# microsoft/vision-longformer

Measured on NVIDIA H100. Metric: images/sec ViL-Small 224x224 training, higher is better.
Workload: dtype bf16

## Files before the change

vision_longformer_b200/csrc/vil_common.cuh:

```cuda
#pragma once
#include <cuda_runtime.h>
#include <cuda_bf16.h>
#include <cuda_fp16.h>
#include <stdint.h>
#include "../../include/vil_attn.h"

namespace vil {

struct Geo {
  int B, H, D;
  int nx, ny, w, g, exact, mode;
  int padx, pady, mx, my;
  int Nloc, N, w2;
  int npc;
  int noffs;
  int offR[9], offC[9];
  int has_bias;
  float scale;
  float drop_p, drop_scale;
  uint32_t drop_thresh;
  uint32_t seed_lo, seed_hi, drop_off;
};

inline long long ws_off_delta_g(const Geo& g) { return ((long long)g.B * g.H * g.Nloc + 63) & ~63LL; }
// ... 62 lines not shown
      return;
    }
  }
#pragma unroll
  for (int c = 0; c < CNT; ++c)
    if (c0 + c < D) row[c0 + c] = ElemTraits<T>::from_f(r[c]);
}

__device__ __forceinline__ uint4 philox(const Geo& g, uint32_t c0, uint32_t c1, uint32_t c2) {
  uint32_t x0 = c0, x1 = c1, x2 = c2, x3 = g.drop_off, k0 = g.seed_lo, k1 = g.seed_hi;
#pragma unroll
  for (int r = 0; r < 10; ++r) {
    const uint32_t lo0 = 0xD2511F53u * x0, hi0 = __umulhi(0xD2511F53u, x0);
    const uint32_t lo1 = 0xCD9E8D57u * x2, hi1 = __umulhi(0xCD9E8D57u, x2);
    x0 = hi1 ^ x1 ^ k0; x1 = lo1; x2 = hi0 ^ x3 ^ k1; x3 = lo0;
    k0 += 0x9E3779B9u; k1 += 0xBB67AE85u;
  }
  return make_uint4(x0, x1, x2, x3);
}
__device__ __forceinline__ uint32_t philox_word(const uint4& x, uint32_t w) {
  return w == 0 ? x.x : w == 1 ? x.y : w == 2 ? x.z : x.w;
}
__device__ __forceinline__ bool drop_keep(const Geo& g, uint32_t row, uint32_t col, uint32_t sid) {
  return philox_word(philox(g, col >> 2, row, sid), col & 3) >= g.drop_thresh;
}
__device__ __forceinline__ void drop_keep2(const Geo& g, uint32_t row, uint32_t col, uint32_t sid, bool& k0, bool& k1) {
  const uint4 x = philox(g, col >> 2, row, sid);
  const uint32_t w = col & 3;
  k0 = philox_word(x, w) >= g.drop_thresh;
  const uint32_t u1 = w == 3 ? philox(g, (col >> 2) + 1, row, sid).x : philox_word(x, w + 1);
  k1 = u1 >= g.drop_thresh;
}

__device__ __forceinline__ float warp_sum(float v) {
#pragma unroll
  for (int o = 16; o > 0; o >>= 1) v += __shfl_xor_sync(0xffffffffu, v, o);
  return v;
}

}
```

vision_longformer_b200/csrc/vil_sm90.cuh:

```cuda
#pragma once
#include <cuda_bf16.h>
#include <cuda_fp16.h>
#include <stdint.h>

namespace sm90 {

__device__ __forceinline__ uint32_t smem_u32(const void* p) { return (uint32_t)__cvta_generic_to_shared(p); }

__host__ __device__ constexpr int core_off(int r, int c, int K) { return (((r >> 3) * (K >> 3) + (c >> 3)) << 6) + ((r & 7) << 3) + (c & 7); }

__device__ __forceinline__ uint64_t make_desc(uint32_t addr, uint32_t lbo, uint32_t sbo) {
  return (uint64_t)((addr >> 4) & 0x3FFF) | (uint64_t)(lbo >> 4) << 16 | (uint64_t)(sbo >> 4) << 32;
}
__device__ __forceinline__ uint64_t desc(const void* tile, int K, int k16) {
  return make_desc(smem_u32(tile) + k16 * 256, 128, (K >> 3) * 128);
}
__device__ __forceinline__ uint64_t desc_mn(const void* tile, int N, int k16) {
  return make_desc(smem_u32(tile) + k16 * N * 32, N * 16, 128);
}

__device__ __forceinline__ void cp_async16(void* dst, const void* src, int n) {
  asm volatile("cp.async.cg.shared.global [%0], [%1], 16, %2;" ::"r"(smem_u32(dst)), "l"(src), "r"(n) : "memory");
}
__device__ __forceinline__ void cp_async4(void* dst, const void* src) {
  asm volatile("cp.async.ca.shared.global [%0], [%1], 4;" ::"r"(smem_u32(dst)), "l"(src) : "memory");
}
__device__ __forceinline__ void cp_async_commit() { asm volatile("cp.async.commit_group;" ::: "memory"); }
template <int N>
__device__ __forceinline__ void cp_async_wait() { asm volatile("cp.async.wait_group %0;" ::"n"(N) : "memory"); }

__device__ __forceinline__ void wg_fence() { asm volatile("wgmma.fence.sync.aligned;" ::: "memory"); }
__device__ __forceinline__ void wg_commit() { asm volatile("wgmma.commit_group.sync.aligned;" ::: "memory"); }
__device__ __forceinline__ void wg_wait0() { asm volatile("wgmma.wait_group.sync.aligned 0;" ::: "memory"); }
__device__ __forceinline__ void fence_proxy_async() { asm volatile("fence.proxy.async.shared::cta;" ::: "memory"); }
template <int R>
__device__ __forceinline__ void reg_fence(float (&d)[R]) {
#pragma unroll
  for (int i = 0; i < R; ++i) asm volatile("" : "+f"(d[i])::"memory");
}

__device__ __forceinline__ void wgmma_ss_bf16_n16(float (&d)[8], uint64_t a, uint64_t b, uint32_t acc) {
  asm volatile(
      "{\n\t.reg .pred p;\n\tsetp.ne.b32 p, %10, 0;\n\t"
      "wgmma.mma_async.sync.aligned.m64n16k16.f32.bf16.bf16 {%0,%1,%2,%3,%4,%5,%6,%7}, %8, %9, p, 1, 1, 0, 0;\n\t}"
      : "+f"(d[0]), "+f"(d[1]), "+f"(d[2]), "+f"(d[3]), "+f"(d[4]), "+f"(d[5]), "+f"(d[6]), "+f"(d[7])
      : "l"(a), "l"(b), "r"(acc));
}
__device__ __forceinline__ void wgmma_rs_bf16_n16(float (&d)[8], const uint32_t (&a)[4], uint64_t b, uint32_t acc) {
  asm volatile(
      "{\n\t.reg .pred p;\n\tsetp.ne.b32 p, %13, 0;\n\t"
      "wgmma.mma_async.sync.aligned.m64n16k16.f32.bf16.bf16 {%0,%1,%2,%3,%4,%5,%6,%7}, {%8,%9,%10,%11}, %12, p, 1, 1, 1;\n\t}"
      : "+f"(d[0]), "+f"(d[1]), "+f"(d[2]), "+f"(d[3]), "+f"(d[4]), "+f"(d[5]), "+f"(d[6]), "+f"(d[7])
      : "r"(a[0]), "r"(a[1]), "r"(a[2]), "r"(a[3]), "l"(b), "r"(acc));
}
__device__ __forceinline__ void wgmma_ss_f16_n16(float (&d)[8], uint64_t a, uint64_t b, uint32_t acc) {
// ... 96 lines not shown
```

vision_longformer_b200/csrc/vil_wgmma.cuh:

```cuda
#pragma once
#include "vil_common.cuh"
#include "vil_sm90.cuh"

namespace vil {
namespace wg {

constexpr int kThreads = 128;

struct Cta { int b, h, R, C, piece; };

__device__ __forceinline__ Cta decode(const Geo& g, int bid) {
  Cta c;
  c.piece = bid % g.npc; bid /= g.npc;
  c.C = bid % g.my; bid /= g.my;
  c.R = bid % g.mx; bid /= g.mx;
  c.h = bid % g.H;
  c.b = bid / g.H;
  return c;
}

__device__ __forceinline__ int acc_row(int i) { return ((threadIdx.x >> 5) << 4) + ((threadIdx.x & 31) >> 2) + (((i >> 1) & 1) << 3); }
__device__ __forceinline__ int acc_col(int i) { return ((i >> 2) << 3) + ((threadIdx.x & 3) << 1) + (i & 1); }

constexpr int kStages = 3;

template <typename T, int HD>
__device__ __forceinline__ void stage_row(T* tile, const T* base, long long st, long long tok, int row, int half, int D) {
  constexpr int HH = HD / 2;
  const T* src = base + (tok < 0 ? 0 : tok * st);
#pragma unroll
  for (int g8 = 0; g8 < HH / 8; ++g8) {
    const int c = half * HH + g8 * 8;
    const bool in = tok >= 0 && c < D;
    sm90::cp_async16(tile + sm90::core_off(row, c, HD), in ? src + c : base, in ? 16 : 0);
  }
}

template <typename T>
__device__ __forceinline__ void to_a_frag(const float (&s)[32], int kk, uint32_t (&a)[4]) {
  a[0] = sm90::pack2<T>(s[8 * kk + 0], s[8 * kk + 1]);
  a[1] = sm90::pack2<T>(s[8 * kk + 2], s[8 * kk + 3]);
  a[2] = sm90::pack2<T>(s[8 * kk + 4], s[8 * kk + 5]);
  a[3] = sm90::pack2<T>(s[8 * kk + 6], s[8 * kk + 7]);
}

template <typename TO, int HD>
__device__ __forceinline__ void store_rows(const float (&acc)[HD / 2], int e, TO* row, int D, float mul) {
  const int c0 = (threadIdx.x & 3) << 1;
#pragma unroll
  for (int j = 0; j < HD / 8; ++j) {
    const int col = 8 * j + c0;
    if (col < D) row[col] = ElemTraits<TO>::from_f(acc[4 * j + 2 * e] * mul);
    if (col + 1 < D) row[col + 1] = ElemTraits<TO>::from_f(acc[4 * j + 2 * e + 1] * mul);
  }
}

__device__ __forceinline__ void drop_key_piece(float (&x)[32], const Geo& geo, const uint32_t (&row)[2], int cbase, uint32_t sid,
                                               float mul) {
  uint32_t keep = 0;
#pragma unroll 1
  for (int i = 0; i < 32; i += 2) {
    bool k0, k1;
    drop_keep2(geo, (i & 2) ? row[1] : row[0], (uint32_t)(cbase + acc_col(i)), sid, k0, k1);
    keep |= ((uint32_t)k0 | ((uint32_t)k1 << 1)) << i;
  }
#pragma unroll
  for (int i = 0; i < 32; ++i) x[i] = (keep >> i) & 1u ? x[i] * mul : 0.f;
}

__device__ __forceinline__ void drop_rows(const Geo& geo, int R, int C, int piece, uint32_t (&row)[2]) {
#pragma unroll
  for (int e = 0; e < 2; ++e) {
    const int l = piece * 64 + acc_row(2 * e);
    row[e] = (uint32_t)((R * geo.w + l / geo.w) * geo.ny + C * geo.w + l % geo.w);
  }
}

struct Visit {
  int r, c;
  int dR, dC;
  int cut;
  int oi;
};

__device__ __forceinline__ int visit_list(const Geo& geo, int R, int C, int sgn, Visit* vl) {
  int n = 0;
  for (int oi = 0; oi < geo.noffs; ++oi) {
    const int dR = geo.offR[oi], dC = geo.offC[oi];
    int r = R + sgn * dR, c = C + sgn * dC;
    if (geo.exact == -1) { r = (r + geo.mx) % geo.mx; c = (c + geo.my) % geo.my; }
    else if (r < 0 || r >= geo.mx || c < 0 || c >= geo.my) continue;
    const int qR = sgn > 0 ? R : r, qC = sgn > 0 ? C : c;
    if (threadIdx.x == 0) vl[n] = Visit{r, c, dR, dC, (qR + dR == geo.mx - 1) | ((qC + dC == geo.my - 1) << 1), oi};
    ++n;
  }
  return n;
}

__device__ __forceinline__ int drop_col_base(const Geo& geo, const Visit* vl, int ngp, int pi) {
  if (pi < ngp) return pi * 64;
  const int vi = (pi - ngp) / geo.npc;
  return geo.g + vl[vi].oi * geo.w2 + (pi - ngp - vi * geo.npc) * 64;
}

struct SlotWalk {
  int vi, pj, kr, kc;
  int r0, c0, dr, dc;
  __device__ __forceinline__ SlotWalk(const Geo& geo, int slot)
      : vi(0), pj(0), r0(slot / geo.w), c0(slot % geo.w), dr(64 / geo.w), dc(64 % geo.w) { kr = r0; kc = c0; }
  __device__ __forceinline__ void next(const Geo& geo) {
    if (++pj == geo.npc) { pj = 0; ++vi; kr = r0; kc = c0; return; }
    kr += dr; kc += dc;
    if (kc >= geo.w) { kc -= geo.w; ++kr; }
  }
};

__device__ __forceinline__ void chunk_key(const Geo& geo, const Visit& v, int kr, int kc, long long& tok, bool& ok, int& vr, int& vc) {
  const int w = geo.w;
  const int ar = v.r * w + kr, ac = v.c * w + kc;
  const bool real = (ar < geo.nx) && (ac < geo.ny);
  if (geo.exact == -1)
    ok = !(((v.cut & 1) && (kr >= w - geo.padx)) || ((v.cut & 2) && (kc >= w - geo.pady)));
  else
    ok = real;
  tok = (ok && real) ? geo.g + (long long)ar * geo.ny + ac : -1;
  vr = v.dR * w + kr; vc = v.dC * w + kc;
}

__device__ __forceinline__ void key_slot(const Geo& geo, const Visit* vl, int ngp, int pi, int slot, SlotWalk& wk, int& gk,
                                         long long& tok, bool& ok, int& vr, int& vc) {
  gk = -1; tok = -1; ok = false; vr = 0; vc = 0;
  if (pi < ngp) {
    const int t = pi * 64 + slot;
    if (t < geo.g) { gk = t; tok = t; ok = true; }
    return;
  }
  if (wk.kr < geo.w) chunk_key(geo, vl[wk.vi], wk.kr, wk.kc, tok, ok, vr, vc);
  wk.next(geo);
}

struct KeyCols {
  float* bias;
  int* tix;
  short* kr;
  short* kc;
};
struct QRows {
  int qr[2], qc[2];
  bool ok[2];
};

__device__ __forceinline__ QRows query_rows(const Geo& geo, int R, int C, int piece) {
  QRows q;
  const int w = geo.w;
#pragma unroll
  for (int e = 0; e < 2; ++e) {
    const int l = piece * 64 + acc_row(2 * e);
    const bool in = l < geo.w2;
    q.qr[e] = in ? l / w : 0; q.qc[e] = in ? l % w : 0;
    q.ok[e] = in && (R * w + q.qr[e] < geo.nx) && (C * w + q.qc[e] < geo.ny);
  }
  return q;
}

__device__ __forceinline__ void stage_key_cols(const Geo& geo, const KeyCols& kc, int h, const float* __restrict__ g2l, int gk,
                                               bool ok, int vr, int vc) {
  const int slot = threadIdx.x >> 1;
  float bias = ok ? 0.f : -INFINITY;
  if (gk >= 0 && geo.has_bias) bias = g2l[((long long)geo.H + h) * geo.g + gk];
  kc.bias[slot] = bias;
  kc.tix[slot] = vr * (4 * geo.w - 1) + vc;
  kc.kr[slot] = (short)vr;
  kc.kc[slot] = (short)vc;
}

__device__ __forceinline__ void row_tix(const Geo& geo, const QRows& q, int (&tb)[2]) {
  const int w = geo.w, tw = 4 * w - 1;
  tb[0] = (q.qr[0] + 2 * w - 1) * tw + q.qc[0] + 2 * w - 1;
  tb[1] = (q.qr[1] + 2 * w - 1) * tw + q.qc[1] + 2 * w - 1;
}

template <bool RPE, bool WIN>
__device__ __forceinline__ float key_score(const Geo& geo, const KeyCols& kc, const float* tab, const QRows& q, const int (&tb)[2],
                                           int e, int j, int gl, float s, int& bidx) {
  float bias = kc.bias[j];
  bidx = -1;
  if (RPE && j >= gl) { bidx = tb[e] - kc.tix[j]; bias += tab[bidx]; }
  if (WIN && (abs(q.qr[e] - kc.kr[j]) > geo.w || abs(q.qc[e] - kc.kc[j]) > geo.w)) return -INFINITY;
  return fmaf(geo.scale, s, bias);
}

__device__ __forceinline__ int key_epilogue(const Geo& geo) { return (geo.has_bias ? 2 : 0) | (geo.exact == 1 ? 1 : 0); }

template <bool RPE, bool WIN>
__device__ __forceinline__ void fwd_scores(float (&s)[32], float (&mx)[2], const Geo& geo, const KeyCols& kc, const float* tab,
                                           const QRows& q, int gl) {
  int tb[2] = {0, 0};
  if (RPE) row_tix(geo, q, tb);
#pragma unroll
  for (int i = 0; i < 32; ++i) {
    const int e = (i >> 1) & 1;
    int bidx;
    s[i] = key_score<RPE, WIN>(geo, kc, tab, q, tb, e, acc_col(i), gl, s[i], bidx);
    mx[e] = fmaxf(mx[e], s[i]);
  }
}

template <bool RPE, bool WIN>
__device__ __forceinline__ void dq_scores(float (&s)[32], const float (&dp)[32], const Geo& geo, const KeyCols& kc,
                                          const float* tab, const QRows& q, int gl, const float (&lse_r)[2],
                                          const float (&del_r)[2], float* __restrict__ d_table, int h) {
  int tb[2] = {0, 0};
  if (RPE) row_tix(geo, q, tb);
#pragma unroll
  for (int i = 0; i < 32; ++i) {
    const int e = (i >> 1) & 1;
    int bidx;
    const float val = key_score<RPE, WIN>(geo, kc, tab, q, tb, e, acc_col(i), gl, s[i], bidx);
    const float ds = __expf(val - lse_r[e]) * (dp[i] - del_r[e]);
    if (RPE && d_table != nullptr && bidx >= 0 && q.ok[e] && val != -INFINITY)
      atomicAdd(d_table + (long long)bidx * geo.H + h, ds);
    s[i] = ds;
  }
}

constexpr size_t kKeyCols = 64 * (4 + 4 + 2 + 2);
constexpr size_t kQueryCols = 64 * (4 + 4 + 4 + 2 + 2 + 1);
constexpr size_t kVisits = 9 * sizeof(Visit);
__host__ __device__ constexpr size_t query_cols_bytes(bool drop) { return kQueryCols + (drop ? 64 * sizeof(int) : 0); }

__device__ __forceinline__ KeyCols key_cols(unsigned char* meta, int stage) {
  KeyCols kc;
  kc.bias = reinterpret_cast<float*>(meta + stage * kKeyCols);
  kc.tix = reinterpret_cast<int*>(kc.bias + 64);
  kc.kr = reinterpret_cast<short*>(kc.tix + 64);
  kc.kc = kc.kr + 64;
  return kc;
}

template <int HD> struct FwdSmem {
  static constexpr size_t tiles = (1 + 2 * kStages) * 64 * HD * 2;
  static size_t total(int tabn) { return (tiles + kStages * kKeyCols + kVisits + (size_t)tabn * 4 + 15) & ~size_t(15); }
};
template <int HD> struct DqSmem {
  static constexpr size_t tiles = (2 + 2 * kStages) * 64 * HD * 2;
  static size_t total(int tabn) { return (tiles + kStages * kKeyCols + kVisits + (size_t)tabn * 4 + 15) & ~size_t(15); }
};
template <int HD> struct DkvSmem {
  static constexpr size_t tiles = (2 + 2 * kStages) * 64 * HD * 2;
  static size_t total(int tabn, bool drop = false) {
    return (tiles + kStages * query_cols_bytes(drop) + kVisits + 64 * sizeof(int) + (size_t)tabn * 4 + 15) & ~size_t(15);
  }
};

template <typename T, int HD>
__device__ __forceinline__ void issue_key_piece(const Geo& geo, int pi, int npieces, int ngp, const Visit* vl, SlotWalk& wk,
                                                T* ring, unsigned char* meta, const T* kb, long long kst, const T* vb,
                                                long long vst, int h, const float* __restrict__ g2l) {
  if (pi < npieces) {
    const int slot = threadIdx.x >> 1, half = threadIdx.x & 1, st = pi % kStages;
    int gk, vr, vc;
    long long tok;
    bool ok;
    key_slot(geo, vl, ngp, pi, slot, wk, gk, tok, ok, vr, vc);
    T* Ks = ring + st * 2 * 64 * HD;
    stage_row<T, HD>(Ks, kb, kst, tok, slot, half, geo.D);
    stage_row<T, HD>(Ks + 64 * HD, vb, vst, tok, slot, half, geo.D);
    if (half == 0) stage_key_cols(geo, key_cols(meta, st), h, g2l, gk, ok, vr, vc);
  }
  sm90::cp_async_commit();
}

__device__ __forceinline__ void ring_wait() {
  sm90::cp_async_wait<kStages - 2>();
  sm90::fence_proxy_async();
  __syncthreads();
}

template <typename T, int HD, typename TO, bool DROP = false>
__global__ void __launch_bounds__(kThreads, HD <= 32 ? 5 : 3)
wg_fwd_local(Geo geo, T4 q, T4 k, T4 v, T4 o, float* __restrict__ lse, const float* __restrict__ table,
             const float* __restrict__ g2l) {
  constexpr int HH = HD / 2, TILE = 64 * HD;
  using W64 = sm90::Wg<T, 64>;
  using WHD = sm90::Wg<T, HD>;
  extern __shared__ __align__(128) unsigned char smem_raw[];
  T* Qs = reinterpret_cast<T*>(smem_raw);
  T* ring = Qs + TILE;
  unsigned char* meta = reinterpret_cast<unsigned char*>(ring + 2 * kStages * TILE);
  Visit* vl = reinterpret_cast<Visit*>(meta + kStages * kKeyCols);
  float* tab = reinterpret_cast<float*>(vl + 9);
  const int tabn = geo.has_bias ? (4 * geo.w - 1) * (4 * geo.w - 1) : 0;

  const Cta cid = decode(geo, blockIdx.x);
  const int b = cid.b, h = cid.h, R = cid.R, C = cid.C;
  const int tid = threadIdx.x, slot = tid >> 1, half = tid & 1;
  const int w = geo.w, D = geo.D;
  for (int i = tid; i < tabn; i += kThreads) tab[i] = table[(long long)i * geo.H + h];
  {
    const int l = cid.piece * 64 + slot;
    const int r = R * w + l / w, c = C * w + l % w;
    const bool real = l < geo.w2 && r < geo.nx && c < geo.ny;
    stage_row<T, HD>(Qs, row_ptr<T>(q, b, h, 0), q.st, real ? (long long)r * geo.ny + c : -1, slot, half, D);
  }
  float m[2] = {-INFINITY, -INFINITY}, lsum[2] = {0.f, 0.f};
  float oacc[HH];
#pragma unroll
  for (int i = 0; i < HH; ++i) oacc[i] = 0.f;

  const int ngp = (geo.g + 63) / 64, npieces = ngp + visit_list(geo, R, C, 1, vl) * geo.npc;
  const int epi = key_epilogue(geo);
  const T* kb = row_ptr<T>(k, b, h, 0);
  const T* vb = row_ptr<T>(v, b, h, 0);
  SlotWalk wk(geo, slot);
  __syncthreads();
#pragma unroll
  for (int p = 0; p < kStages - 1; ++p)
    issue_key_piece<T, HD>(geo, p, npieces, ngp, vl, wk, ring, meta, kb, k.st, vb, v.st, h, g2l);
  for (int pi = 0; pi < npieces; ++pi) {
    ring_wait();
    issue_key_piece<T, HD>(geo, pi + kStages - 1, npieces, ngp, vl, wk, ring, meta, kb, k.st, vb, v.st, h, g2l);
    const int st = pi % kStages;
    const T* Ks = ring + st * 2 * TILE;
    const T* Vs = Ks + TILE;
    const KeyCols kcol = key_cols(meta, st);
    float s[32];
    sm90::wg_fence();
#pragma unroll
    for (int kk = 0; kk < HD / 16; ++kk) W64::ss(s, sm90::desc(Qs, HD, kk), sm90::desc(Ks, HD, kk), kk > 0);
    sm90::wg_commit();
    sm90::wg_wait0();
    sm90::reg_fence(s);
    float mx[2] = {-INFINITY, -INFINITY};
    const int gl = geo.g - pi * 64;
    switch (epi) {
      case 0: fwd_scores<false, false>(s, mx, geo, kcol, tab, query_rows(geo, R, C, cid.piece), gl); break;
      case 1: fwd_scores<false, true>(s, mx, geo, kcol, tab, query_rows(geo, R, C, cid.piece), gl); break;
      case 2: fwd_scores<true, false>(s, mx, geo, kcol, tab, query_rows(geo, R, C, cid.piece), gl); break;
      default: fwd_scores<true, true>(s, mx, geo, kcol, tab, query_rows(geo, R, C, cid.piece), gl); break;
    }
    float corr[2];
#pragma unroll
    for (int e = 0; e < 2; ++e) {
      mx[e] = fmaxf(mx[e], __shfl_xor_sync(0xffffffffu, mx[e], 1));
      mx[e] = fmaxf(mx[e], __shfl_xor_sync(0xffffffffu, mx[e], 2));
      const float mn = fmaxf(m[e], mx[e]);
      corr[e] = (mn == -INFINITY) ? 1.f : __expf(m[e] - mn);
      m[e] = mn;
      lsum[e] *= corr[e];
    }
#pragma unroll
    for (int i = 0; i < 32; ++i) {
      const int e = (i >> 1) & 1;
      const float p = (m[e] == -INFINITY) ? 0.f : __expf(s[i] - m[e]);
      s[i] = p;
      lsum[e] += p;
    }
#pragma unroll
    for (int i = 0; i < HH; ++i) oacc[i] *= corr[(i >> 1) & 1];
    if constexpr (DROP) {
      uint32_t drow[2];
      drop_rows(geo, R, C, cid.piece, drow);
      drop_key_piece(s, geo, drow, drop_col_base(geo, vl, ngp, pi), 2u * (uint32_t)(b * geo.H + h), 1.f);
    }
    uint32_t a[4][4];
#pragma unroll
    for (int kk = 0; kk < 4; ++kk) to_a_frag<T>(s, kk, a[kk]);
    sm90::wg_fence();
#pragma unroll
    for (int kk = 0; kk < 4; ++kk) WHD::rs(oacc, a[kk], sm90::desc_mn(Vs, HD, kk), 1);
    sm90::wg_commit();
    sm90::wg_wait0();
    sm90::reg_fence(oacc);
  }
  const QRows qrow = query_rows(geo, R, C, cid.piece);
#pragma unroll
  for (int e = 0; e < 2; ++e) {
    lsum[e] += __shfl_xor_sync(0xffffffffu, lsum[e], 1);
    lsum[e] += __shfl_xor_sync(0xffffffffu, lsum[e], 2);
    if (!qrow.ok[e]) continue;
    const long long tokq = (long long)(R * w + qrow.qr[e]) * geo.ny + (C * w + qrow.qc[e]);
    const float inv = lsum[e] > 0.f ? 1.f / lsum[e] : 0.f;
    store_rows<TO, HD>(oacc, e, row_ptr_w<TO>(o, b, h, tokq), D, DROP ? inv * geo.drop_scale : inv);
    if ((tid & 3) == 0) lse[((long long)b * geo.H + h) * geo.Nloc + tokq] = m[e] + logf(lsum[e]);
  }
}

template <typename T, int HD, typename TO, bool DROP = false>
__global__ void __launch_bounds__(kThreads)
wg_bwd_dq(Geo geo, T4 q, T4 k, T4 v, T4 d_o, T4 dq, const float* __restrict__ lse, const float* __restrict__ delta,
          const float* __restrict__ table, const float* __restrict__ g2l, float* __restrict__ d_table) {
  constexpr int HH = HD / 2, TILE = 64 * HD;
  using W64 = sm90::Wg<T, 64>;
  using WHD = sm90::Wg<T, HD>;
  extern __shared__ __align__(128) unsigned char smem_raw[];
  T* Qs = reinterpret_cast<T*>(smem_raw);
  T* Gs = Qs + TILE;
  T* ring = Gs + TILE;
  unsigned char* meta = reinterpret_cast<unsigned char*>(ring + 2 * kStages * TILE);
  Visit* vl = reinterpret_cast<Visit*>(meta + kStages * kKeyCols);
  float* tab = reinterpret_cast<float*>(vl + 9);
  const int tabn = geo.has_bias ? (4 * geo.w - 1) * (4 * geo.w - 1) : 0;

  const Cta cid = decode(geo, blockIdx.x);
  const int b = cid.b, h = cid.h, R = cid.R, C = cid.C;
  const int tid = threadIdx.x, slot = tid >> 1, half = tid & 1;
  const int w = geo.w, D = geo.D;
  const long long bh = (long long)b * geo.H + h;
  for (int i = tid; i < tabn; i += kThreads) tab[i] = table[(long long)i * geo.H + h];
  {
    const int l = cid.piece * 64 + slot;
    const int r = R * w + l / w, c = C * w + l % w;
    const long long tokq = (l < geo.w2 && r < geo.nx && c < geo.ny) ? (long long)r * geo.ny + c : -1;
    stage_row<T, HD>(Qs, row_ptr<T>(q, b, h, 0), q.st, tokq, slot, half, D);
    stage_row<T, HD>(Gs, row_ptr<T>(d_o, b, h, 0), d_o.st, tokq, slot, half, D);
  }
  const QRows qrow = query_rows(geo, R, C, cid.piece);
  float lse_r[2], del_r[2];
#pragma unroll
  for (int e = 0; e < 2; ++e) {
    lse_r[e] = INFINITY; del_r[e] = 0.f;
    if (qrow.ok[e]) {
      const long long tokq = (long long)(R * w + qrow.qr[e]) * geo.ny + (C * w + qrow.qc[e]);
      lse_r[e] = lse[bh * geo.Nloc + tokq];
      del_r[e] = delta[bh * geo.Nloc + tokq];
    }
  }
  float dqacc[HH];
#pragma unroll
  for (int i = 0; i < HH; ++i) dqacc[i] = 0.f;

  const int ngp = (geo.g + 63) / 64, npieces = ngp + visit_list(geo, R, C, 1, vl) * geo.npc;
  const int epi = key_epilogue(geo);
  const T* kb = row_ptr<T>(k, b, h, 0);
  const T* vb = row_ptr<T>(v, b, h, 0);
  SlotWalk wk(geo, slot);
  __syncthreads();
#pragma unroll
  for (int p = 0; p < kStages - 1; ++p)
    issue_key_piece<T, HD>(geo, p, npieces, ngp, vl, wk, ring, meta, kb, k.st, vb, v.st, h, g2l);
  for (int pi = 0; pi < npieces; ++pi) {
    ring_wait();
    issue_key_piece<T, HD>(geo, pi + kStages - 1, npieces, ngp, vl, wk, ring, meta, kb, k.st, vb, v.st, h, g2l);
    const int st = pi % kStages;
    const T* Ks = ring + st * 2 * TILE;
    const T* Vs = Ks + TILE;
    const KeyCols kcol = key_cols(meta, st);
    float s[32], dp[32];
    sm90::wg_fence();
#pragma unroll
    for (int kk = 0; kk < HD / 16; ++kk) W64::ss(s, sm90::desc(Qs, HD, kk), sm90::desc(Ks, HD, kk), kk > 0);
#pragma unroll
    for (int kk = 0; kk < HD / 16; ++kk) W64::ss(dp, sm90::desc(Gs, HD, kk), sm90::desc(Vs, HD, kk), kk > 0);
    sm90::wg_commit();
    sm90::wg_wait0();
    sm90::reg_fence(s);
    sm90::reg_fence(dp);
    const int gl = geo.g - pi * 64;
    if constexpr (DROP) {
      uint32_t drow[2];
      drop_rows(geo, R, C, cid.piece, drow);
      drop_key_piece(dp, geo, drow, drop_col_base(geo, vl, ngp, pi), 2u * (uint32_t)(b * geo.H + h), geo.drop_scale);
    }
    switch (epi) {
      case 0: dq_scores<false, false>(s, dp, geo, kcol, tab, qrow, gl, lse_r, del_r, d_table, h); break;
      case 1: dq_scores<false, true>(s, dp, geo, kcol, tab, qrow, gl, lse_r, del_r, d_table, h); break;
      case 2: dq_scores<true, false>(s, dp, geo, kcol, tab, qrow, gl, lse_r, del_r, d_table, h); break;
      default: dq_scores<true, true>(s, dp, geo, kcol, tab, qrow, gl, lse_r, del_r, d_table, h); break;
    }
    uint32_t a[4][4];
#pragma unroll
    for (int kk = 0; kk < 4; ++kk) to_a_frag<T>(s, kk, a[kk]);
    sm90::wg_fence();
#pragma unroll
    for (int kk = 0; kk < 4; ++kk) WHD::rs(dqacc, a[kk], sm90::desc_mn(Ks, HD, kk), 1);
    sm90::wg_commit();
    sm90::wg_wait0();
    sm90::reg_fence(dqacc);
  }
#pragma unroll
  for (int e = 0; e < 2; ++e) {
    if (!qrow.ok[e]) continue;
    const long long tokq = (long long)(R * w + qrow.qr[e]) * geo.ny + (C * w + qrow.qc[e]);
    store_rows<TO, HD>(dqacc, e, row_ptr_w<TO>(dq, b, h, tokq), D, geo.scale);
  }
}

// ... 15 lines not shown

__device__ __forceinline__ int key_pos(const Geo& geo, int piece, int row) {
  const int lk = piece * 64 + row;
  return lk < geo.w2 ? (lk / geo.w) | ((lk % geo.w) << 8) | (1 << 16) : 0;
}

__device__ __forceinline__ KRows key_rows(const Geo& geo, int KR, int KC, const int* kpos) {
  KRows k;
  const int w = geo.w, tw = 4 * w - 1;
#pragma unroll
  for (int e = 0; e < 2; ++e) {
    const int pos = kpos[acc_row(2 * e)];
    const bool in = pos >> 16;
    k.kr[e] = pos & 0xff; k.kc[e] = (pos >> 8) & 0xff;
    k.real[e] = in && (KR * w + k.kr[e] < geo.nx) && (KC * w + k.kc[e] < geo.ny);
    k.tb[e] = k.kr[e] * tw + k.kc[e] - (2 * w - 1) * (tw + 1);
    k.cut[e] = (k.kr[e] >= w - geo.padx) | ((k.kc[e] >= w - geo.pady) << 1);
  }
  return k;
}

__device__ __forceinline__ QueryCols query_cols(unsigned char* meta, int stage, int bytes) {
  QueryCols qc;
  qc.lse = reinterpret_cast<float*>(meta + stage * bytes);
  qc.del = qc.lse + 64;
  qc.tix = reinterpret_cast<int*>(qc.del + 64);
  qc.qr = reinterpret_cast<short*>(qc.tix + 64);
  qc.qc = qc.qr + 64;
  qc.cut = reinterpret_cast<unsigned char*>(qc.qc + 64);
  qc.tok = reinterpret_cast<int*>(qc.cut + 64);
  return qc;
}

template <typename T, int HD, bool DROP>
__device__ __forceinline__ void issue_query_piece(const Geo& geo, int qp, int npieces, const Visit* vl, SlotWalk& wk, T* ring,
                                                  unsigned char* meta, const T* qb, long long qst, const T* gb, long long gst,
                                                  const float* __restrict__ lse, const float* __restrict__ delta) {
  if (qp < npieces) {
    const int slot = threadIdx.x >> 1, half = threadIdx.x & 1, st = qp % kStages, w = geo.w;
    bool qv = false;
    long long tq = 0;
    int qa = 0, qb2 = 0, cut = 0;
    if (wk.kr < w) {
      const Visit vq = vl[wk.vi];
      const int r = vq.r * w + wk.kr, c = vq.c * w + wk.kc;
      qv = (r < geo.nx) && (c < geo.ny);
      tq = (long long)r * geo.ny + c;
      qa = wk.kr - vq.dR * w; qb2 = wk.kc - vq.dC * w; cut = vq.cut;
    }
    wk.next(geo);
    T* Qs = ring + st * 2 * 64 * HD;
    stage_row<T, HD>(Qs, qb, qst, qv ? tq : -1, slot, half, geo.D);
    stage_row<T, HD>(Qs + 64 * HD, gb, gst, qv ? tq : -1, slot, half, geo.D);
    if (half == 0) {
      const QueryCols qcol = query_cols(meta, st, (int)query_cols_bytes(DROP));
      if (qv) {
        sm90::cp_async4(qcol.lse + slot, lse + tq);
        sm90::cp_async4(qcol.del + slot, delta + tq);
      } else {
        qcol.lse[slot] = INFINITY;
        qcol.del[slot] = 0.f;
      }
      const int tw = 4 * w - 1;
      qcol.tix[slot] = qa * tw + qb2;
      qcol.qr[slot] = (short)qa; qcol.qc[slot] = (short)qb2;
      qcol.cut[slot] = (unsigned char)cut;
      if (DROP) qcol.tok[slot] = (int)tq;
    }
  }
  sm90::cp_async_commit();
}

__device__ __forceinline__ int query_epilogue(const Geo& geo) {
  return (geo.has_bias ? 3 : 0) + (geo.exact == 1 ? 1 : geo.exact == -1 ? 2 : 0);
}

template <bool RPE, int MASK>
__device__ __forceinline__ void dkv_probs(float (&s)[32], float (&dp)[32], const Geo& geo, const QueryCols& qc, const float* tab,
                                          const KRows& kr) {
#pragma unroll
  for (int i = 0; i < 32; ++i) {
    const int e = (i >> 1) & 1, j = acc_col(i);
    float x = fmaf(geo.scale, s[i], RPE ? tab[qc.tix[j] - kr.tb[e]] : 0.f) - qc.lse[j];
    if (MASK == 1 && (abs(qc.qr[j] - kr.kr[e]) > geo.w || abs(qc.qc[j] - kr.kc[e]) > geo.w)) x = -INFINITY;
    if (MASK == 2 && (qc.cut[j] & kr.cut[e])) x = -INFINITY;
    const float p = __expf(x);
    s[i] = p;
    dp[i] = p * (dp[i] - qc.del[j]);
  }
}

template <typename T, int HD, typename TO, bool DROP = false>
__global__ void __launch_bounds__(kThreads, (HD <= 32 ? 4 : 3) - (DROP ? 1 : 0))
wg_bwd_dkv(Geo geo, T4 q, T4 k, T4 v, T4 d_o, T4 dk, T4 dv, const float* __restrict__ lse, const float* __restrict__ delta,
           const float* __restrict__ table) {
  constexpr int HH = HD / 2, TILE = 64 * HD;
  using W64 = sm90::Wg<T, 64>;
  using WHD = sm90::Wg<T, HD>;
  extern __shared__ __align__(128) unsigned char smem_raw[];
  T* Ks = reinterpret_cast<T*>(smem_raw);
  T* Vs = Ks + TILE;
  T* ring = Vs + TILE;
  unsigned char* meta = reinterpret_cast<unsigned char*>(ring + 2 * kStages * TILE);
  const int cols = (int)query_cols_bytes(DROP);
  Visit* vl = reinterpret_cast<Visit*>(meta + kStages * cols);
  int* kpos = reinterpret_cast<int*>(vl + 9);
  float* tab = reinterpret_cast<float*>(kpos + 64);
  const int tw = 4 * geo.w - 1;
  const int tabn = geo.has_bias ? tw * tw : 0;

  const Cta cid = decode(geo, blockIdx.x);
  const int b = cid.b, h = cid.h, KR = cid.R, KC = cid.C;
  const int tid = threadIdx.x, slot = tid >> 1, half = tid & 1;
  const int w = geo.w, D = geo.D;
  const long long bh = (long long)b * geo.H + h;
  for (int i = tid; i < tabn; i += kThreads) tab[i] = table[(long long)i * geo.H + h];
  {
    const int lk = cid.piece * 64 + slot;
    const int ar = KR * w + lk / w, ac = KC * w + lk % w;
    const long long tokk = (lk < geo.w2 && ar < geo.nx && ac < geo.ny) ? geo.g + (long long)ar * geo.ny + ac : -1;
    stage_row<T, HD>(Ks, row_ptr<T>(k, b, h, 0), k.st, tokk, slot, half, D);
    stage_row<T, HD>(Vs, row_ptr<T>(v, b, h, 0), v.st, tokk, slot, half, D);
    if (half == 0) kpos[slot] = key_pos(geo, cid.piece, slot);
  }
  float dkacc[HH], dvacc[HH];
#pragma unroll
  for (int i = 0; i < HH; ++i) { dkacc[i] = 0.f; dvacc[i] = 0.f; }

  const int npieces = visit_list(geo, KR, KC, -1, vl) * geo.npc;
  const int epi = query_epilogue(geo);
  SlotWalk wk(geo, slot);
  __syncthreads();
#pragma unroll
  for (int p = 0; p < kStages - 1; ++p)
    issue_query_piece<T, HD, DROP>(geo, p, npieces, vl, wk, ring, meta, row_ptr<T>(q, b, h, 0), q.st,
                                   row_ptr<T>(d_o, b, h, 0), d_o.st, lse + bh * geo.Nloc, delta + bh * geo.Nloc);
  for (int qp = 0; qp < npieces; ++qp) {
    ring_wait();
    issue_query_piece<T, HD, DROP>(geo, qp + kStages - 1, npieces, vl, wk, ring, meta, row_ptr<T>(q, b, h, 0), q.st,
                                   row_ptr<T>(d_o, b, h, 0), d_o.st, lse + bh * geo.Nloc, delta + bh * geo.Nloc);
    const int st = qp % kStages;
    const T* Qs = ring + st * 2 * TILE;
    const T* Gs = Qs + TILE;
    const QueryCols qcol = query_cols(meta, st, cols);
    uint32_t keep = 0;
    if constexpr (DROP) {
      const int vi = qp / geo.npc;
      const uint32_t c0 = (uint32_t)(geo.g + vl[vi].oi * geo.w2 + cid.piece * 64), sid = 2u * (uint32_t)(b * geo.H + h);
#pragma unroll 1
      for (int i = 0; i < 32; ++i)
        keep |= (uint32_t)drop_keep(geo, (uint32_t)qcol.tok[acc_col(i)], c0 + (uint32_t)acc_row(i), sid) << i;
    }
    float s[32], dp[32];
    sm90::wg_fence();
#pragma unroll
    for (int kk = 0; kk < HD / 16; ++kk) W64::ss(s, sm90::desc(Ks, HD, kk), sm90::desc(Qs, HD, kk), kk > 0);
#pragma unroll
    for (int kk = 0; kk < HD / 16; ++kk) W64::ss(dp, sm90::desc(Vs, HD, kk), sm90::desc(Gs, HD, kk), kk > 0);
    sm90::wg_commit();
    sm90::wg_wait0();
    sm90::reg_fence(s);
    sm90::reg_fence(dp);
    if constexpr (DROP) {
#pragma unroll
      for (int i = 0; i < 32; ++i) dp[i] = (keep >> i) & 1u ? dp[i] * geo.drop_scale : 0.f;
    }
    switch (epi) {
      case 0: dkv_probs<false, 0>(s, dp, geo, qcol, tab, key_rows(geo, KR, KC, kpos)); break;
      case 1: dkv_probs<false, 1>(s, dp, geo, qcol, tab, key_rows(geo, KR, KC, kpos)); break;
      case 2: dkv_probs<false, 2>(s, dp, geo, qcol, tab, key_rows(geo, KR, KC, kpos)); break;
      case 3: dkv_probs<true, 0>(s, dp, geo, qcol, tab, key_rows(geo, KR, KC, kpos)); break;
      case 4: dkv_probs<true, 1>(s, dp, geo, qcol, tab, key_rows(geo, KR, KC, kpos)); break;
      default: dkv_probs<true, 2>(s, dp, geo, qcol, tab, key_rows(geo, KR, KC, kpos)); break;
    }
    if constexpr (DROP) {
#pragma unroll
      for (int i = 0; i < 32; ++i) s[i] = (keep >> i) & 1u ? s[i] * geo.drop_scale : 0.f;
    }
    uint32_t ap[4][4], ad[4][4];
#pragma unroll
    for (int kk = 0; kk < 4; ++kk) { to_a_frag<T>(s, kk, ap[kk]); to_a_frag<T>(dp, kk, ad[kk]); }
    sm90::wg_fence();
#pragma unroll
    for (int kk = 0; kk < 4; ++kk) WHD::rs(dvacc, ap[kk], sm90::desc_mn(Gs, HD, kk), 1);
#pragma unroll
    for (int kk = 0; kk < 4; ++kk) WHD::rs(dkacc, ad[kk], sm90::desc_mn(Qs, HD, kk), 1);
    sm90::wg_commit();
    sm90::wg_wait0();
    sm90::reg_fence(dvacc);
    sm90::reg_fence(dkacc);
  }
  const KRows krow = key_rows(geo, KR, KC, kpos);
// ... 12 lines not shown
```

Measured before the change: 4545.

## Overlap next-piece cp.async issue with WGMMA and simplify staging address math

Moves the prefetch of the next K/V (or Q/dO) ring stage to after the WGMMA commit so address computation and cp.async issue overlap the tensor-core work. It also precomputes per-visit token bases and bounds, replaces the stage_row helper with a RowSeg that uses precomputed shared-memory addresses, writes only the metadata the current epilogue needs, swaps __expf for ex2.approx.ftz, and adds a minBlocks launch bound to the dQ kernel. The cost targeted is the per-piece integer overhead and the serialization between copy issue and MMA. In exchange, the 32-bit token indices and ftz exponent could differ in edge cases, and the new launch bound may cause register spills.

Result: faster. 4653, median of 6 (+2.4%).

```diff
diff --git a/vision_longformer_b200/csrc/vil_common.cuh b/vision_longformer_b200/csrc/vil_common.cuh
--- a/vision_longformer_b200/csrc/vil_common.cuh
+++ b/vision_longformer_b200/csrc/vil_common.cuh
@@ -118,6 +118,12 @@
   k1 = u1 >= g.drop_thresh;
 }
 
+__device__ __forceinline__ float exp_ftz(float x) {
+  float y;
+  asm("ex2.approx.ftz.f32 %0, %1;" : "=f"(y) : "f"(__fmul_rn(x, 1.44269504f)));
+  return y;
+}
+
 __device__ __forceinline__ float warp_sum(float v) {
 #pragma unroll
   for (int o = 16; o > 0; o >>= 1) v += __shfl_xor_sync(0xffffffffu, v, o);
diff --git a/vision_longformer_b200/csrc/vil_sm90.cuh b/vision_longformer_b200/csrc/vil_sm90.cuh
--- a/vision_longformer_b200/csrc/vil_sm90.cuh
+++ b/vision_longformer_b200/csrc/vil_sm90.cuh
@@ -19,8 +19,8 @@
   return make_desc(smem_u32(tile) + k16 * N * 32, N * 16, 128);
 }
 
-__device__ __forceinline__ void cp_async16(void* dst, const void* src, int n) {
-  asm volatile("cp.async.cg.shared.global [%0], [%1], 16, %2;" ::"r"(smem_u32(dst)), "l"(src), "r"(n) : "memory");
+__device__ __forceinline__ void cp_async16(uint32_t dst, const void* src, int n) {
+  asm volatile("cp.async.cg.shared.global [%0], [%1], 16, %2;" ::"r"(dst), "l"(src), "r"(n) : "memory");
 }
 __device__ __forceinline__ void cp_async4(void* dst, const void* src) {
   asm volatile("cp.async.ca.shared.global [%0], [%1], 4;" ::"r"(smem_u32(dst)), "l"(src) : "memory");
diff --git a/vision_longformer_b200/csrc/vil_wgmma.cuh b/vision_longformer_b200/csrc/vil_wgmma.cuh
--- a/vision_longformer_b200/csrc/vil_wgmma.cuh
+++ b/vision_longformer_b200/csrc/vil_wgmma.cuh
@@ -25,16 +25,20 @@
 constexpr int kStages = 3;
 
 template <typename T, int HD>
-__device__ __forceinline__ void stage_row(T* tile, const T* base, long long st, long long tok, int row, int half, int D) {
-  constexpr int HH = HD / 2;
-  const T* src = base + (tok < 0 ? 0 : tok * st);
-#pragma unroll
-  for (int g8 = 0; g8 < HH / 8; ++g8) {
-    const int c = half * HH + g8 * 8;
-    const bool in = tok >= 0 && c < D;
-    sm90::cp_async16(tile + sm90::core_off(row, c, HD), in ? src + c : base, in ? 16 : 0);
-  }
-}
+struct RowSeg {
+  uint32_t dst;
+  int col;
+  __device__ __forceinline__ RowSeg(int slot, int half)
+      : dst((uint32_t)(sm90::core_off(slot, half * (HD / 2), HD) * sizeof(T))), col(half * (HD / 2)) {}
+  __device__ __forceinline__ void copy(uint32_t tile, const T* base, long long st, int tok, bool valid, int D) const {
+    const T* row = base + (long long)(unsigned)(valid ? tok : 0) * st;
+#pragma unroll
+    for (int g8 = 0; g8 < HD / 16; ++g8) {
+      const bool in = col + 8 * g8 < D;
+      sm90::cp_async16(tile + dst + 128 * g8, in ? row + col + 8 * g8 : row, valid && in ? 16 : 0);
+    }
+  }
+};
 
 template <typename T>
 __device__ __forceinline__ void to_a_frag(const float (&s)[32], int kk, uint32_t (&a)[4]) {
@@ -77,13 +81,16 @@
 }
 
 struct Visit {
-  int r, c;
-  int dR, dC;
+  int tok;
+  int nr, nc;
+  int mr, mc;
+  int dRw, dCw;
   int cut;
   int oi;
 };
 
 __device__ __forceinline__ int visit_list(const Geo& geo, int R, int C, int sgn, Visit* vl) {
+  const int w = geo.w;
   int n = 0;
   for (int oi = 0; oi < geo.noffs; ++oi) {
     const int dR = geo.offR[oi], dC = geo.offC[oi];
@@ -91,7 +98,15 @@
     if (geo.exact == -1) { r = (r + geo.mx) % geo.mx; c = (c + geo.my) % geo.my; }
     else if (r < 0 || r >= geo.mx || c < 0 || c >= geo.my) continue;
     const int qR = sgn > 0 ? R : r, qC = sgn > 0 ? C : c;
-    if (threadIdx.x == 0) vl[n] = Visit{r, c, dR, dC, (qR + dR == geo.mx - 1) | ((qC + dC == geo.my - 1) << 1), oi};
+    const int cut = (qR + dR == geo.mx - 1) | ((qC + dC == geo.my - 1) << 1);
+    int nr = min(w, geo.nx - r * w), nc = min(w, geo.ny - c * w), mr = nr, mc = nc;
+    if (sgn > 0 && geo.exact == -1) {
+      mr = (cut & 1) ? w - geo.padx : w;
+      mc = (cut & 2) ? w - geo.pady : w;
+      nr = min(nr, mr); nc = min(nc, mc);
+    }
+    if (threadIdx.x == 0)
+      vl[n] = Visit{(sgn > 0 ? geo.g : 0) + r * w * geo.ny + c * w, nr, nc, mr, mc, dR * w, dC * w, cut, oi};
     ++n;
   }
   return n;
@@ -115,27 +130,21 @@
   }
 };
 
-__device__ __forceinline__ void chunk_key(const Geo& geo, const Visit& v, int kr, int kc, long long& tok, bool& ok, int& vr, int& vc) {
-  const int w = geo.w;
-  const int ar = v.r * w + kr, ac = v.c * w + kc;
-  const bool real = (ar < geo.nx) && (ac < geo.ny);
-  if (geo.exact == -1)
-    ok = !(((v.cut & 1) && (kr >= w - geo.padx)) || ((v.cut & 2) && (kc >= w - geo.pady)));
-  else
-    ok = real;
-  tok = (ok && real) ? geo.g + (long long)ar * geo.ny + ac : -1;
-  vr = v.dR * w + kr; vc = v.dC * w + kc;
-}
-
 __device__ __forceinline__ void key_slot(const Geo& geo, const Visit* vl, int ngp, int pi, int slot, SlotWalk& wk, int& gk,
-                                         long long& tok, bool& ok, int& vr, int& vc) {
-  gk = -1; tok = -1; ok = false; vr = 0; vc = 0;
+                                         int& tok, bool& real, bool& ok, int& vr, int& vc) {
+  gk = -1; tok = 0; real = false; ok = false; vr = 0; vc = 0;
   if (pi < ngp) {
     const int t = pi * 64 + slot;
-    if (t < geo.g) { gk = t; tok = t; ok = true; }
+    if (t < geo.g) { gk = t; tok = t; real = true; ok = true; }
     return;
   }
-  if (wk.kr < geo.w) chunk_key(geo, vl[wk.vi], wk.kr, wk.kc, tok, ok, vr, vc);
+  if (wk.kr < geo.w) {
+    const Visit& v = vl[wk.vi];
+    tok = v.tok + wk.kr * geo.ny + wk.kc;
+    real = wk.kr < v.nr && wk.kc < v.nc;
+    ok = wk.kr < v.mr && wk.kc < v.mc;
+    vr = v.dRw + wk.kr; vc = v.dCw + wk.kc;
+  }
   wk.next(geo);
 }
 
@@ -163,15 +172,14 @@
   return q;
 }
 
-__device__ __forceinline__ void stage_key_cols(const Geo& geo, const KeyCols& kc, int h, const float* __restrict__ g2l, int gk,
-                                               bool ok, int vr, int vc) {
+__device__ __forceinline__ void stage_key_cols(const Geo& geo, const KeyCols& kc, int epi, int h, const float* __restrict__ g2l,
+                                               int gk, bool ok, int vr, int vc) {
   const int slot = threadIdx.x >> 1;
   float bias = ok ? 0.f : -INFINITY;
   if (gk >= 0 && geo.has_bias) bias = g2l[((long long)geo.H + h) * geo.g + gk];
   kc.bias[slot] = bias;
-  kc.tix[slot] = vr * (4 * geo.w - 1) + vc;
-  kc.kr[slot] = (short)vr;
-  kc.kc[slot] = (short)vc;
+  if (epi & 2) kc.tix[slot] = vr * (4 * geo.w - 1) + vc;
+  if (epi & 1) { kc.kr[slot] = (short)vr; kc.kc[slot] = (short)vc; }
 }
 
 __device__ __forceinline__ void row_tix(const Geo& geo, const QRows& q, int (&tb)[2]) {
@@ -217,7 +225,7 @@
     const int e = (i >> 1) & 1;
     int bidx;
     const float val = key_score<RPE, WIN>(geo, kc, tab, q, tb, e, acc_col(i), gl, s[i], bidx);
-    const float ds = __expf(val - lse_r[e]) * (dp[i] - del_r[e]);
+    const float ds = exp_ftz(val - lse_r[e]) * (dp[i] - del_r[e]);
     if (RPE && d_table != nullptr && bidx >= 0 && q.ok[e] && val != -INFINITY)
       atomicAdd(d_table + (long long)bidx * geo.H + h, ds);
     s[i] = ds;
@@ -254,19 +262,18 @@
 };
 
 template <typename T, int HD>
-__device__ __forceinline__ void issue_key_piece(const Geo& geo, int pi, int npieces, int ngp, const Visit* vl, SlotWalk& wk,
-                                                T* ring, unsigned char* meta, const T* kb, long long kst, const T* vb,
-                                                long long vst, int h, const float* __restrict__ g2l) {
+__device__ __forceinline__ void issue_key_piece(const Geo& geo, int pi, int st, int npieces, int ngp, int epi, const Visit* vl,
+                                                SlotWalk& wk, const RowSeg<T, HD>& seg, uint32_t tiles, unsigned char* meta,
+                                                const T* kb, long long kst, const T* vb, long long vst, int h,
+                                                const float* __restrict__ g2l) {
   if (pi < npieces) {
-    const int slot = threadIdx.x >> 1, half = threadIdx.x & 1, st = pi % kStages;
-    int gk, vr, vc;
-    long long tok;
-    bool ok;
-    key_slot(geo, vl, ngp, pi, slot, wk, gk, tok, ok, vr, vc);
-    T* Ks = ring + st * 2 * 64 * HD;
-    stage_row<T, HD>(Ks, kb, kst, tok, slot, half, geo.D);
-    stage_row<T, HD>(Ks + 64 * HD, vb, vst, tok, slot, half, geo.D);
-    if (half == 0) stage_key_cols(geo, key_cols(meta, st), h, g2l, gk, ok, vr, vc);
+    const int slot = threadIdx.x >> 1;
+    int gk, tok, vr, vc;
+    bool real, ok;
+    key_slot(geo, vl, ngp, pi, slot, wk, gk, tok, real, ok, vr, vc);
+    seg.copy(tiles, kb, kst, tok, real, geo.D);
+    seg.copy(tiles + 64 * HD * sizeof(T), vb, vst, tok, real, geo.D);
+    if ((threadIdx.x & 1) == 0) stage_key_cols(geo, key_cols(meta, st), epi, h, g2l, gk, ok, vr, vc);
   }
   sm90::cp_async_commit();
 }
@@ -276,6 +283,9 @@
   sm90::fence_proxy_async();
   __syncthreads();
 }
+
+__device__ __forceinline__ int next_stage(int st) { return st == kStages - 1 ? 0 : st + 1; }
+__device__ __forceinline__ int prev_stage(int st) { return st == 0 ? kStages - 1 : st - 1; }
 
 template <typename T, int HD, typename TO, bool DROP = false>
 __global__ void __launch_bounds__(kThreads, HD <= 32 ? 5 : 3)
@@ -297,11 +307,11 @@
   const int tid = threadIdx.x, slot = tid >> 1, half = tid & 1;
   const int w = geo.w, D = geo.D;
   for (int i = tid; i < tabn; i += kThreads) tab[i] = table[(long long)i * geo.H + h];
+  const RowSeg<T, HD> seg(slot, half);
   {
     const int l = cid.piece * 64 + slot;
     const int r = R * w + l / w, c = C * w + l % w;
-    const bool real = l < geo.w2 && r < geo.nx && c < geo.ny;
-    stage_row<T, HD>(Qs, row_ptr<T>(q, b, h, 0), q.st, real ? (long long)r * geo.ny + c : -1, slot, half, D);
+    seg.copy(sm90::smem_u32(Qs), row_ptr<T>(q, b, h, 0), q.st, r * geo.ny + c, l < geo.w2 && r < geo.nx && c < geo.ny, D);
   }
   float m[2] = {-INFINITY, -INFINITY}, lsum[2] = {0.f, 0.f};
   float oacc[HH];
@@ -312,15 +322,15 @@
   const int epi = key_epilogue(geo);
   const T* kb = row_ptr<T>(k, b, h, 0);
   const T* vb = row_ptr<T>(v, b, h, 0);
+  constexpr uint32_t kStageBytes = 2 * TILE * sizeof(T);
+  const uint32_t ring_a = sm90::smem_u32(ring);
   SlotWalk wk(geo, slot);
   __syncthreads();
 #pragma unroll
   for (int p = 0; p < kStages - 1; ++p)
-    issue_key_piece<T, HD>(geo, p, npieces, ngp, vl, wk, ring, meta, kb, k.st, vb, v.st, h, g2l);
-  for (int pi = 0; pi < npieces; ++pi) {
+    issue_key_piece<T, HD>(geo, p, p, npieces, ngp, epi, vl, wk, seg, ring_a + p * kStageBytes, meta, kb, k.st, vb, v.st, h, g2l);
+  for (int pi = 0, st = 0; pi < npieces; ++pi, st = next_stage(st)) {
     ring_wait();
-    issue_key_piece<T, HD>(geo, pi + kStages - 1, npieces, ngp, vl, wk, ring, meta, kb, k.st, vb, v.st, h, g2l);
-    const int st = pi % kStages;
     const T* Ks = ring + st * 2 * TILE;
     const T* Vs = Ks + TILE;
     const KeyCols kcol = key_cols(meta, st);
@@ -329,6 +339,8 @@
 #pragma unroll
     for (int kk = 0; kk < HD / 16; ++kk) W64::ss(s, sm90::desc(Qs, HD, kk), sm90::desc(Ks, HD, kk), kk > 0);
     sm90::wg_commit();
+    issue_key_piece<T, HD>(geo, pi + kStages - 1, prev_stage(st), npieces, ngp, epi, vl, wk, seg,
+                           ring_a + prev_stage(st) * kStageBytes, meta, kb, k.st, vb, v.st, h, g2l);
     sm90::wg_wait0();
     sm90::reg_fence(s);
     float mx[2] = {-INFINITY, -INFINITY};
@@ -339,20 +351,21 @@
       case 2: fwd_scores<true, false>(s, mx, geo, kcol, tab, query_rows(geo, R, C, cid.piece), gl); break;
       default: fwd_scores<true, true>(s, mx, geo, kcol, tab, query_rows(geo, R, C, cid.piece), gl); break;
     }
-    float corr[2];
+    float corr[2], mu[2];
 #pragma unroll
     for (int e = 0; e < 2; ++e) {
       mx[e] = fmaxf(mx[e], __shfl_xor_sync(0xffffffffu, mx[e], 1));
       mx[e] = fmaxf(mx[e], __shfl_xor_sync(0xffffffffu, mx[e], 2));
       const float mn = fmaxf(m[e], mx[e]);
-      corr[e] = (mn == -INFINITY) ? 1.f : __expf(m[e] - mn);
+      corr[e] = (mn == -INFINITY) ? 1.f : exp_ftz(m[e] - mn);
       m[e] = mn;
+      mu[e] = (mn == -INFINITY) ? 0.f : mn;
       lsum[e] *= corr[e];
     }
 #pragma unroll
     for (int i = 0; i < 32; ++i) {
       const int e = (i >> 1) & 1;
-      const float p = (m[e] == -INFINITY) ? 0.f : __expf(s[i] - m[e]);
+      const float p = exp_ftz(s[i] - mu[e]);
       s[i] = p;
       lsum[e] += p;
     }
@@ -387,7 +400,7 @@
 }
 
 template <typename T, int HD, typename TO, bool DROP = false>
-__global__ void __launch_bounds__(kThreads)
+__global__ void __launch_bounds__(kThreads, DROP ? 3 : HD <= 32 ? 4 : 3)
 wg_bwd_dq(Geo geo, T4 q, T4 k, T4 v, T4 d_o, T4 dq, const float* __restrict__ lse, const float* __restrict__ delta,
           const float* __restrict__ table, const float* __restrict__ g2l, float* __restrict__ d_table) {
   constexpr int HH = HD / 2, TILE = 64 * HD;
@@ -408,12 +421,13 @@
   const int w = geo.w, D = geo.D;
   const long long bh = (long long)b * geo.H + h;
   for (int i = tid; i < tabn; i += kThreads) tab[i] = table[(long long)i * geo.H + h];
+  const RowSeg<T, HD> seg(slot, half);
   {
     const int l = cid.piece * 64 + slot;
     const int r = R * w + l / w, c = C * w + l % w;
-    const long long tokq = (l < geo.w2 && r < geo.nx && c < geo.ny) ? (long long)r * geo.ny + c : -1;
-    stage_row<T, HD>(Qs, row_ptr<T>(q, b, h, 0), q.st, tokq, slot, half, D);
-    stage_row<T, HD>(Gs, row_ptr<T>(d_o, b, h, 0), d_o.st, tokq, slot, half, D);
+    const bool real = l < geo.w2 && r < geo.nx && c < geo.ny;
+    seg.copy(sm90::smem_u32(Qs), row_ptr<T>(q, b, h, 0), q.st, r * geo.ny + c, real, D);
+    seg.copy(sm90::smem_u32(Gs), row_ptr<T>(d_o, b, h, 0), d_o.st, r * geo.ny + c, real, D);
   }
   const QRows qrow = query_rows(geo, R, C, cid.piece);
   float lse_r[2], del_r[2];
@@ -434,15 +448,15 @@
   const int epi = key_epilogue(geo);
   const T* kb = row_ptr<T>(k, b, h, 0);
   const T* vb = row_ptr<T>(v, b, h, 0);
+  constexpr uint32_t kStageBytes = 2 * TILE * sizeof(T);
+  const uint32_t ring_a = sm90::smem_u32(ring);
   SlotWalk wk(geo, slot);
   __syncthreads();
 #pragma unroll
   for (int p = 0; p < kStages - 1; ++p)
-    issue_key_piece<T, HD>(geo, p, npieces, ngp, vl, wk, ring, meta, kb, k.st, vb, v.st, h, g2l);
-  for (int pi = 0; pi < npieces; ++pi) {
+    issue_key_piece<T, HD>(geo, p, p, npieces, ngp, epi, vl, wk, seg, ring_a + p * kStageBytes, meta, kb, k.st, vb, v.st, h, g2l);
+  for (int pi = 0, st = 0; pi < npieces; ++pi, st = next_stage(st)) {
     ring_wait();
-    issue_key_piece<T, HD>(geo, pi + kStages - 1, npieces, ngp, vl, wk, ring, meta, kb, k.st, vb, v.st, h, g2l);
-    const int st = pi % kStages;
     const T* Ks = ring + st * 2 * TILE;
     const T* Vs = Ks + TILE;
     const KeyCols kcol = key_cols(meta, st);
@@ -453,6 +467,8 @@
 #pragma unroll
     for (int kk = 0; kk < HD / 16; ++kk) W64::ss(dp, sm90::desc(Gs, HD, kk), sm90::desc(Vs, HD, kk), kk > 0);
     sm90::wg_commit();
+    issue_key_piece<T, HD>(geo, pi + kStages - 1, prev_stage(st), npieces, ngp, epi, vl, wk, seg,
+                           ring_a + prev_stage(st) * kStageBytes, meta, kb, k.st, vb, v.st, h, g2l);
     sm90::wg_wait0();
     sm90::reg_fence(s);
     sm90::reg_fence(dp);
@@ -534,27 +550,24 @@
   return qc;
 }
 
+__device__ __forceinline__ int query_epilogue(const Geo& geo) {
+  return (geo.has_bias ? 3 : 0) + (geo.exact == 1 ? 1 : geo.exact == -1 ? 2 : 0);
+}
+
 template <typename T, int HD, bool DROP>
-__device__ __forceinline__ void issue_query_piece(const Geo& geo, int qp, int npieces, const Visit* vl, SlotWalk& wk, T* ring,
-                                                  unsigned char* meta, const T* qb, long long qst, const T* gb, long long gst,
+__device__ __forceinline__ void issue_query_piece(const Geo& geo, int qp, int st, int npieces, int epi, const Visit* vl,
+                                                  SlotWalk& wk, const RowSeg<T, HD>& seg, uint32_t tiles, unsigned char* meta,
+                                                  const T* qb, long long qst, const T* gb, long long gst,
                                                   const float* __restrict__ lse, const float* __restrict__ delta) {
   if (qp < npieces) {
-    const int slot = threadIdx.x >> 1, half = threadIdx.x & 1, st = qp % kStages, w = geo.w;
-    bool qv = false;
-    long long tq = 0;
-    int qa = 0, qb2 = 0, cut = 0;
-    if (wk.kr < w) {
-      const Visit vq = vl[wk.vi];
-      const int r = vq.r * w + wk.kr, c = vq.c * w + wk.kc;
-      qv = (r < geo.nx) && (c < geo.ny);
-      tq = (long long)r * geo.ny + c;
-      qa = wk.kr - vq.dR * w; qb2 = wk.kc - vq.dC * w; cut = vq.cut;
-    }
-    wk.next(geo);
-    T* Qs = ring + st * 2 * 64 * HD;
-    stage_row<T, HD>(Qs, qb, qst, qv ? tq : -1, slot, half, geo.D);
-    stage_row<T, HD>(Qs + 64 * HD, gb, gst, qv ? tq : -1, slot, half, geo.D);
-    if (half == 0) {
+    const int slot = threadIdx.x >> 1;
+    const bool in = wk.kr < geo.w;
+    const Visit& vq = vl[wk.vi];
+    const bool qv = wk.kr < vq.nr && wk.kc < vq.nc;
+    const int tq = vq.tok + wk.kr * geo.ny + wk.kc;
+    seg.copy(tiles, qb, qst, tq, qv, geo.D);
+    seg.copy(tiles + 64 * HD * sizeof(T), gb, gst, tq, qv, geo.D);
+    if ((threadIdx.x & 1) == 0) {
       const QueryCols qcol = query_cols(meta, st, (int)query_cols_bytes(DROP));
       if (qv) {
         sm90::cp_async4(qcol.lse + slot, lse + tq);
@@ -563,18 +576,15 @@
         qcol.lse[slot] = INFINITY;
         qcol.del[slot] = 0.f;
       }
-      const int tw = 4 * w - 1;
-      qcol.tix[slot] = qa * tw + qb2;
-      qcol.qr[slot] = (short)qa; qcol.qc[slot] = (short)qb2;
-      qcol.cut[slot] = (unsigned char)cut;
-      if (DROP) qcol.tok[slot] = (int)tq;
-    }
+      const int qa = in ? wk.kr - vq.dRw : 0, qb2 = in ? wk.kc - vq.dCw : 0, mask = epi % 3;
+      if (epi >= 3) qcol.tix[slot] = qa * (4 * geo.w - 1) + qb2;
+      if (mask == 1) { qcol.qr[slot] = (short)qa; qcol.qc[slot] = (short)qb2; }
+      if (mask == 2) qcol.cut[slot] = (unsigned char)(in ? vq.cut : 0);
+      if (DROP) qcol.tok[slot] = in ? tq : 0;
+    }
+    wk.next(geo);
   }
   sm90::cp_async_commit();
-}
-
-__device__ __forceinline__ int query_epilogue(const Geo& geo) {
-  return (geo.has_bias ? 3 : 0) + (geo.exact == 1 ? 1 : geo.exact == -1 ? 2 : 0);
 }
 
 template <bool RPE, int MASK>
@@ -586,7 +596,7 @@
     float x = fmaf(geo.scale, s[i], RPE ? tab[qc.tix[j] - kr.tb[e]] : 0.f) - qc.lse[j];
     if (MASK == 1 && (abs(qc.qr[j] - kr.kr[e]) > geo.w || abs(qc.qc[j] - kr.kc[e]) > geo.w)) x = -INFINITY;
     if (MASK == 2 && (qc.cut[j] & kr.cut[e])) x = -INFINITY;
-    const float p = __expf(x);
+    const float p = exp_ftz(x);
     s[i] = p;
     dp[i] = p * (dp[i] - qc.del[j]);
   }
@@ -617,12 +627,13 @@
   const int w = geo.w, D = geo.D;
   const long long bh = (long long)b * geo.H + h;
   for (int i = tid; i < tabn; i += kThreads) tab[i] = table[(long long)i * geo.H + h];
+  const RowSeg<T, HD> seg(slot, half);
   {
     const int lk = cid.piece * 64 + slot;
     const int ar = KR * w + lk / w, ac = KC * w + lk % w;
-    const long long tokk = (lk < geo.w2 && ar < geo.nx && ac < geo.ny) ? geo.g + (long long)ar * geo.ny + ac : -1;
-    stage_row<T, HD>(Ks, row_ptr<T>(k, b, h, 0), k.st, tokk, slot, half, D);
-    stage_row<T, HD>(Vs, row_ptr<T>(v, b, h, 0), v.st, tokk, slot, half, D);
+    const bool real = lk < geo.w2 && ar < geo.nx && ac < geo.ny;
+    seg.copy(sm90::smem_u32(Ks), row_ptr<T>(k, b, h, 0), k.st, geo.g + ar * geo.ny + ac, real, D);
+    seg.copy(sm90::smem_u32(Vs), row_ptr<T>(v, b, h, 0), v.st, geo.g + ar * geo.ny + ac, real, D);
     if (half == 0) kpos[slot] = key_pos(geo, cid.piece, slot);
   }
   float dkacc[HH], dvacc[HH];
@@ -631,16 +642,16 @@
 
   const int npieces = visit_list(geo, KR, KC, -1, vl) * geo.npc;
   const int epi = query_epilogue(geo);
+  constexpr uint32_t kStageBytes = 2 * TILE * sizeof(T);
+  const uint32_t ring_a = sm90::smem_u32(ring);
   SlotWalk wk(geo, slot);
   __syncthreads();
 #pragma unroll
   for (int p = 0; p < kStages - 1; ++p)
-    issue_query_piece<T, HD, DROP>(geo, p, npieces, vl, wk, ring, meta, row_ptr<T>(q, b, h, 0), q.st,
-                                   row_ptr<T>(d_o, b, h, 0), d_o.st, lse + bh * geo.Nloc, delta + bh * geo.Nloc);
+    issue_query_piece<T, HD, DROP>(geo, p, p, npieces, epi, vl, wk, seg, ring_a + p * kStageBytes, meta, row_ptr<T>(q, b, h, 0),
+                                   q.st, row_ptr<T>(d_o, b, h, 0), d_o.st, lse + bh * geo.Nloc, delta + bh * geo.Nloc);
   for (int qp = 0; qp < npieces; ++qp) {
     ring_wait();
-    issue_query_piece<T, HD, DROP>(geo, qp + kStages - 1, npieces, vl, wk, ring, meta, row_ptr<T>(q, b, h, 0), q.st,
-                                   row_ptr<T>(d_o, b, h, 0), d_o.st, lse + bh * geo.Nloc, delta + bh * geo.Nloc);
     const int st = qp % kStages;
     const T* Qs = ring + st * 2 * TILE;
     const T* Gs = Qs + TILE;
@@ -660,6 +671,12 @@
 #pragma unroll
     for (int kk = 0; kk < HD / 16; ++kk) W64::ss(dp, sm90::desc(Vs, HD, kk), sm90::desc(Gs, HD, kk), kk > 0);
     sm90::wg_commit();
+    {
+      const int sn = (qp + kStages - 1) % kStages;
+      issue_query_piece<T, HD, DROP>(geo, qp + kStages - 1, sn, npieces, epi, vl, wk, seg, ring_a + sn * kStageBytes, meta,
+                                     row_ptr<T>(q, b, h, 0), q.st, row_ptr<T>(d_o, b, h, 0), d_o.st, lse + bh * geo.Nloc,
+                                     delta + bh * geo.Nloc);
+    }
     sm90::wg_wait0();
     sm90::reg_fence(s);
     sm90::reg_fence(dp);
```
